# scaleoutsystems/multimodal-MoE

Hardware: AMD Instinct MI355X
Metric: images/sec (fwd+bwd) RT-DETR-MoE 1280×720 bs=8/GPU at 1/2/4/8 MI355X (higher is better)
Workload: dtype bf16; 1 GPU; C2: RT-DETR-R50 + 8-expert top-2 MoE, bs=8/GPU, bf16; arch=rtdetr-r50-moe8-top2, global_batch=8, execution=hipGraph: forward + criterion (GPU matcher) + backward, precision=bf16 weights + fp32 master, img=1280x720 (padded to 1280x736), parallelism=dp1, batch=8

## Files before the change

### include/moe_hip.h

```cpp
#ifndef MOE_HIP_H_
#define MOE_HIP_H_

#include <stdint.h>
#include <hip/hip_runtime_api.h>

#ifdef __cplusplus
extern "C" {
#endif

int moe_router_num_blocks(int T);

int moe_router_topk_fwd(const void* x, const float* wg, const float* ctx_bias,
                        const int32_t* ctx_img, int n_ctx, int tokens_per_image,
                        int T, int d, int E, int k, int normalize,
                        int32_t* topk_idx, float* topk_w, float* probs, float* lse,
                        int32_t* local_rank, int32_t* block_counts,
                        float* aux_partials, hipStream_t stream);

int moe_route_scan(const int32_t* block_counts, int nblk, int k, int E, int cap,
                   int32_t* rank_base, int32_t* hist, int32_t* offsets,
                   hipStream_t stream);

int moe_permute_fwd(const void* x, const int32_t* topk_idx, const int32_t* local_rank,
                    const int32_t* rank_base, const int32_t* offsets,
// ... 298 lines not shown
int rtdetr_conv_fwd_act(const void* x, const void* w, void* y, const void* zero, int B, int H, int W, int C, int N,
                        int KS, int stride, const float* bias, const void* resid, int act, int resid_post,
                        long long y_img_rows, long long y_row_off, hipStream_t stream);
int rtdetr_conv_fwd_stats_rows(int B, int H, int W, int C, int N, int KS, int stride);
int rtdetr_conv_fwd_stats(const void* x, const void* w, void* y, const void* zero, int B, int H, int W, int C,
                          int N, int KS, int stride, float* part, hipStream_t stream);
long long rtdetr_conv_dgrad_workspace(int B, int H, int W, int C, int N, int KS);
int rtdetr_conv_dgrad(const void* dy, const void* w, void* work, void* dx, const void* zero, int B, int H, int W,
                      int C, int N, int KS, int stride, const void* add, const void* relu_mask, hipStream_t stream);
int rtdetr_conv_weight_flip_multi(const void* table, int n, int total_blocks, hipStream_t stream);
int rtdetr_conv_dgrad_preflipped(const void* dy, const void* w, const void* wflip, void* dx, const void* zero, int B,
                                 int H, int W, int C, int N, int KS, int stride, const void* add, const void* relu_mask,
                                 hipStream_t stream);
int rtdetr_conv_wgrad_splits(int B, int H, int W, int C, int N, int KS);
int rtdetr_conv_wgrad(const void* dy, const void* x, float* part, int nsplit, void* dw, int out_bf16,
                      const void* zero, int B, int H, int W, int C, int N, int KS, int stride, hipStream_t stream);
int rtdetr_conv_wgrad_part(const void* dy, const void* x, float* part, int nsplit, const void* zero, int B, int H,
                           int W, int C, int N, int KS, int stride, hipStream_t stream);
int rtdetr_conv_wgrad_reduce_batch(int n, const float* const* parts, const int* nsplits, const long long* nws,
                                   void* const* dws, int out_bf16, hipStream_t stream);
int rtdetr_conv1x1_bwd(const void* dy, const void* x, const void* w, void* dx, float* part, int nsplit,
                       const void* zero, int B, int H, int W, int C, int N, const void* add, int mask_input,
                       hipStream_t stream);
int rtdetr_conv_set_tuning(const char* key, int value);

int train_grad_pack(const void* tensors, const int32_t* chunks, int n_chunks, float* flat, hipStream_t stream);
int train_grad_sqnorm(const void* tensors, const int32_t* chunks, int n_chunks, float* partials,
                      hipStream_t stream);
int train_grad_norm_finalize(const float* partials, int n, float max_norm, float inv_world, float* coef,
                             const void* tensors, int n_tensors, int32_t* tensor_steps, hipStream_t stream);
int train_adamw_step(const void* tensors, const int32_t* chunks, int n_chunks, const float* coef,
                     float* master, float* exp_avg, float* exp_avg_sq, const int32_t* tensor_steps,
                     const float* lrs, int n_groups, float weight_decay, float beta1, float beta2, float eps,
                     hipStream_t stream);

int train_adamw_ema_step(const void* tensors, const int32_t* chunks, int n_chunks, const float* coef,
                         float* master, float* exp_avg, float* exp_avg_sq, const int32_t* tensor_steps,
                         const float* lrs, int n_groups, float weight_decay, float beta1, float beta2, float eps,
                         float* ema, float ema_decay, hipStream_t stream);
int train_ema_update(const void* tensors, const int32_t* chunks, int n_chunks, float* ema, float ema_decay,
                     hipStream_t stream);

int train_grad_accum(const void* tensors, const int32_t* chunks, int n_chunks, float* acc, int first,
                     hipStream_t stream);

int train_augment_images(const void* src, int src_dtype, long long sn, long long sc, long long sh, long long sw,
// ... 53 lines not shown
```

### multimodal-moe_amd/csrc/conv.hip

```cpp
#include <algorithm>

#include "mfma_lds.h"
#include "moe_common.h"
#include "prof.h"

namespace moe {

static int wg_bm(int N) { return N % 128 == 0 ? 128 : 64; }
static int wg_bn(int C) { return C % 128 == 0 ? 128 : 64; }
static int g_conv_bm = 0;
static int g_conv_big = 0;
static int g_conv_wg_stages = 0;
static int g_conv_wg_splits = 0;
static int g_conv_dgrad_flip = -1;
static int g_conv_dgrad_phase = 1;
static int g_conv_areg = 0;
static int g_conv_halo = -1;
static int g_conv_8ph = -1;
static int g_conv_k32 = -1;

struct ConvArgs {
  const uint16_t* x;
  const uint16_t* w;
  uint16_t* y;
// ... 1242 lines not shown
          const uint32_t lo = mw[q] & 0xffffu, hi = mw[q] >> 16;
          const uint32_t keep_lo = ((lo & 0x8000u) || lo == 0) ? 0u : 0xffffu;
          const uint32_t keep_hi = ((hi & 0x8000u) || hi == 0) ? 0u : 0xffff0000u;
          vw[q] &= keep_lo | keep_hi;
        }
        v = make_uint4(vw[0], vw[1], vw[2], vw[3]);
      }
      const long long p = p0 + r;
      if (p < a.P) *reinterpret_cast<uint4*>(a.dx + (size_t)p * C + xs * 64 + (lane & 7) * 8) = v;
    }
    rslot = rslot + 1 == S ? 0 : rslot + 1;
    islot = islot + 1 == S ? 0 : islot + 1;
  }
#pragma unroll
  for (int i = 0; i < 4; ++i) {
    float* row = out + (size_t)(64 * nb + 16 * i + (lane & 15)) * C + 64 * cb + 4 * (lane >> 4);
#pragma unroll
    for (int j = 0; j < 4; ++j)
      *reinterpret_cast<float4*>(row + 16 * j) =
          make_float4(accw[i][j][0], accw[i][j][1], accw[i][j][2], accw[i][j][3]);
  }
}

template <auto FN>
static void allow_lds_once(size_t bytes) {
  static unsigned long long done = 0;
  (void)allow_dyn_lds(reinterpret_cast<const void*>(FN), (int)bytes, &done, "conv: dynamic LDS");
}

static int conv_out(int n, int KS, int stride) { return (n + 2 * ((KS - 1) / 2) - KS) / stride + 1; }

static int conv_check(const void* const* ptrs, int np, int B, int H, int W, int C, int N, int KS, int stride,
                      const char* what, int cmul = 64) {
  if (KS != 1 && KS != 3) return fail(std::string(what) + ": kernel size must be 1 or 3");
  if (stride != 1 && !(stride == 2 && KS == 3)) return fail(std::string(what) + ": stride must be 1 (or 2 with KS 3)");
  if (B < 0 || H <= 0 || W <= 0) return fail(std::string(what) + ": bad B / H / W");
  if (C % cmul || N % cmul || C <= 0 || N <= 0)
    return fail(std::string(what) + ": channels must be positive multiples of " + std::to_string(cmul));
  if ((long long)B * H * W * (C > N ? C : N) >= (1ll << 31)) return fail(std::string(what) + ": tensor too large");
  for (int i = 0; i < np; ++i)
    if (ptrs[i] == nullptr || reinterpret_cast<uintptr_t>(ptrs[i]) % 16)
      return fail(std::string(what) + ": operands must be non-NULL and 16-B aligned");
  return 0;
}

constexpr int CV_STAGES = 2;
// ... 448 lines not shown
  if (int rc = conv_check(ptrs, 6, B, H, W, C, N, 1, 1, "rtdetr_conv1x1_bwd")) return rc;
  if (!((C == 64 && N == 256) || (C == 256 && N == 64)))
    return fail("rtdetr_conv1x1_bwd: takes {C, N} = {64, 256} (the ResNet stage-1 1x1 layers)");
  if (!aligned16(add)) return fail("rtdetr_conv1x1_bwd: add must be 16-B aligned");
  if (nsplit < 1 || nsplit > 256) return fail("rtdetr_conv1x1_bwd: nsplit must be 1..256");
  Conv1x1BwdArgs a{static_cast<const uint16_t*>(dy), static_cast<const uint16_t*>(x), static_cast<const uint16_t*>(w),
                   static_cast<uint16_t*>(dx), part, static_cast<const uint16_t*>(add),
                   static_cast<const uint16_t*>(zero), B * H * W, 0, mask_input ? 1 : 0};
  const int ktot = (a.P + 63) / 64;
  a.kt_per = (ktot + nsplit - 1) / nsplit;
  const double P = a.P, nw = (double)N * C;
  ProfScope prof(stream, PROF_CONV, 2.0 * P * (N + 2 * C + (add ? C : 0)) + 2.0 * nw + 4.0 * nsplit * nw, false, 0.0,
                 4.0 * P * nw);
  if (C == 64) {
    if (add) launch_conv1x1_bwd<64, 256, true>(a, nsplit, stream, prof);
    else launch_conv1x1_bwd<64, 256, false>(a, nsplit, stream, prof);
  } else {
    if (add) launch_conv1x1_bwd<256, 64, true>(a, nsplit, stream, prof);
    else launch_conv1x1_bwd<256, 64, false>(a, nsplit, stream, prof);
  }
  return check_launch("rtdetr_conv1x1_bwd");
}

extern "C" int rtdetr_conv3x3_direct_fwd(const void* x, const float* wf, const float* bias, void* y, int B, int H,
                                         int W, int C, int N, int stride, int relu, hipStream_t stream) {
  if (C != 3 || N != 32) return fail("rtdetr_conv3x3_direct_fwd: takes C = 3 -> N = 32 (the ResNet-D stem)");
  if (stride != 1 && stride != 2) return fail("rtdetr_conv3x3_direct_fwd: stride 1 or 2");
  if (B < 0 || H <= 0 || W <= 0) return fail("rtdetr_conv3x3_direct_fwd: bad B / H / W");
  if (B == 0) return 0;
  if (x == nullptr || wf == nullptr || y == nullptr || reinterpret_cast<uintptr_t>(y) % 16)
    return fail("rtdetr_conv3x3_direct_fwd: x, wf non-NULL, y 16-B aligned");
  const int Ho = conv_out(H, 3, stride), Wo = conv_out(W, 3, stride);
  const long long P = (long long)B * Ho * Wo;
  const long long blocks = (P + 255) / 256;
  if (blocks > 0x7fffffffLL) return fail("rtdetr_conv3x3_direct_fwd: too many pixels");
  ProfScope prof(stream, PROF_CONV, 2.0 * ((double)B * H * W * C + P * N), false, 0.0, 2.0 * P * N * 9 * C);
  MOE_LAUNCH(prof, (conv_direct_kernel<32, 3>), dim3((unsigned)blocks), dim3(256), 0, stream,
             static_cast<const uint16_t*>(x), wf, bias, static_cast<uint16_t*>(y), B, H, W, Ho, Wo, stride, relu);
  return check_launch("rtdetr_conv3x3_direct_fwd");
}

extern "C" int rtdetr_conv_set_tuning(const char* key, int value) {
  if (key == nullptr) return fail("rtdetr_conv_set_tuning: key is NULL");
  if (std::string(key) == "conv_bm") {
    g_conv_bm = value;
    return 0;
// ... 41 lines not shown
```

### multimodal-moe_amd/src/moe/_lib.py

```python
from __future__ import annotations

import ctypes
import os
from pathlib import Path

import torch

_PKG = Path(__file__).resolve().parents[2]
LIB_PATH = Path(os.environ.get("MOE_HIP_LIB", _PKG / "lib" / "libmoe_hip.so"))

MOE_BF16 = 0
MOE_FP8_E4M3 = 1
MOE_BIAS_BF16 = 0x100
MOE_DENSE_LAYER = 0x200
EPI_NONE, EPI_BIAS, EPI_BIAS_RELU, EPI_RELU_MASK, EPI_RELU_MASK_MX = 0, 1, 2, 3, 4
MX_BLOCK = 32

_P = ctypes.c_void_p
_I = ctypes.c_int
_F = ctypes.c_float
_LL = ctypes.c_longlong
SIGNATURES = {
    "moe_router_num_blocks": (_I, [_I]),
    "moe_router_topk_fwd": (_I, [_P, _P, _P, _P, _I, _I, _I, _I, _I, _I, _I, _P, _P, _P, _P, _P, _P, _P, _P]),
# ... 93 lines not shown
                             _I, _I, _I, _I, _F, _P]),
    "rtdetr_attn_fwd_seg": (_I, [_P, _LL, _P, _LL, _P, _LL, _P, _LL, _P, _I, _I, _I, _I, _F, _P, _P]),
    "rtdetr_attn_bwd_seg": (_I, [_P, _LL, _P, _LL, _P, _LL, _P, _LL, _P, _LL, _P, _P, _P, _LL, _P, _LL, _P, _LL,
                                 _I, _I, _I, _I, _F, _P, _P]),
    "rtdetr_conv_fwd": (_I, [_P, _P, _P, _P, _I, _I, _I, _I, _I, _I, _I, _P, _P, _I, _P]),
    "rtdetr_conv_fwd_act": (_I, [_P, _P, _P, _P, _I, _I, _I, _I, _I, _I, _I, _P, _P, _I, _I, _LL, _LL, _P]),
    "rtdetr_conv_fwd_stats_rows": (_I, [_I, _I, _I, _I, _I, _I, _I]),
    "rtdetr_conv_fwd_stats": (_I, [_P, _P, _P, _P, _I, _I, _I, _I, _I, _I, _I, _P, _P]),
    "rtdetr_bn_act_fwd_part": (_I, [_P, _P, _P, _P, _P, _I, ctypes.c_longlong, _I, _I, _F, _F, _P, _I, _P, _P, _P]),
    "rtdetr_bn_act_fwd_rows": (_I, [_P, _P, _P, _P, _P, _I, ctypes.c_longlong, _I, _I, _F, _F, _P, _I, _P, _P, _P,
                                    _P, ctypes.c_longlong, ctypes.c_longlong, _P]),
    "rtdetr_bn_act_bwd_rows": (_I, [_P, ctypes.c_longlong, ctypes.c_longlong, _P, _P, _I, ctypes.c_longlong, _I, _I,
                                    _P, _P, _P, _P, _P, _P]),
    "rtdetr_conv_dgrad_workspace": (_LL, [_I, _I, _I, _I, _I, _I]),
    "rtdetr_conv_dgrad": (_I, [_P, _P, _P, _P, _P, _I, _I, _I, _I, _I, _I, _I, _P, _P, _P]),
    "rtdetr_conv_dgrad_preflipped": (_I, [_P, _P, _P, _P, _P, _I, _I, _I, _I, _I, _I, _I, _P, _P, _P]),
    "rtdetr_conv_weight_flip_multi": (_I, [_P, _I, _I, _P]),
    "rtdetr_conv_wgrad_splits": (_I, [_I, _I, _I, _I, _I, _I]),
    "rtdetr_conv_set_tuning": (_I, [ctypes.c_char_p, _I]),
    "rtdetr_conv_wgrad": (_I, [_P, _P, _P, _I, _P, _I, _P, _I, _I, _I, _I, _I, _I, _I, _P]),
    "rtdetr_conv_wgrad_part": (_I, [_P, _P, _P, _I, _P, _I, _I, _I, _I, _I, _I, _I, _P]),
    "rtdetr_conv_wgrad_reduce_batch": (_I, [_I, _P, _P, _P, _P, _I, _P]),
    "rtdetr_conv1x1_bwd": (_I, [_P, _P, _P, _P, _P, _I, _P, _I, _I, _I, _I, _I, _P, _I, _P]),
    "train_grad_pack": (_I, [_P, _P, _I, _P, _P]),
    "train_grad_accum": (_I, [_P, _P, _I, _P, _I, _P]),
    "train_grad_sqnorm": (_I, [_P, _P, _I, _P, _P]),
    "train_grad_norm_finalize": (_I, [_P, _I, _F, _F, _P, _P, _I, _P, _P]),
    "train_adamw_step": (_I, [_P, _P, _I, _P, _P, _P, _P, _P, _P, _I, _F, _F, _F, _F, _P]),
    "train_adamw_ema_step": (_I, [_P, _P, _I, _P, _P, _P, _P, _P, _P, _I, _F, _F, _F, _F, _P, _F, _P]),
    "train_ema_update": (_I, [_P, _P, _I, _P, _F, _P]),
    "train_augment_images": (_I, [_P, _I, _LL, _LL, _LL, _LL, _P, _I, _P, _I, _I, _I, _I, _I, _F, _P]),
    "train_augment_boxes": (_I, [_P, _P, _P, _P, _I, _I, _I, _I, _I, _I, _P, _P, _P, _P, _P]),
    "train_mosaic_images": (_I, [_P, _I, _LL, _LL, _LL, _LL, _I, _P, _I, _P, _I, _I, _I, _I, _I, _F, _P]),
    "train_mosaic_boxes": (_I, [_P, _P, _P, _P, _I, _I, _I, _I, _I, _I, _I, _P, _P, _P, _P, _P]),
    "moe_profile_enable": (_I, [_I]),
    "moe_profile_count": (_I, []),
    "moe_profile_get": (_I, [_I, _P, _P, _P, _P]),
    "moe_profile_clear": (_I, []),
    "moe_expert_ffn_bwd": (_I, [_P, _P, _P, _P, _P, _P, _P, _P, _I, _I, _I, _I, _P, _P, _P, _P, _P, _P, _I, _P]),
    "moe_launch_counts": (_I, [_P, _I]),
    "moe_launch_counts_reset": (_I, []),
    "moe_last_error": (ctypes.c_char_p, []),
    "moe_version": (ctypes.c_char_p, []),
}


# ... 1343 lines not shown
```

### multimodal-moe_amd/src/rtdetr_moe/backbone.py

```python
from __future__ import annotations

import ctypes
import os

import torch
from torch import nn
import torch.nn.functional as F

from .conv import conv2d, conv2d_add_bias_relu_fork, conv2d_bias_relu, conv_module, conv_module_stats, hip_conv_ok_for
from .fused import AddBiasReLU, AddBiasReLUFork, BiasReLU, bn_act, bn_act_eval, bn_act_ok, bn_eval_ok

_FUSED_BN = os.environ.get("MOE_FUSED_BN", "1") != "0"
_FUSED_EPI = os.environ.get("MOE_CONV_EPI", "1") != "0"

_DEPTHS = {18: [2, 2, 2, 2], 34: [3, 4, 6, 3], 50: [3, 4, 6, 3], 101: [3, 4, 23, 3]}


class FrozenBatchNorm2d(nn.Module):

    def __init__(self, n, eps=1e-5):
        super().__init__()
        self.register_buffer("weight", torch.ones(n))
        self.register_buffer("bias", torch.zeros(n))
        self.register_buffer("running_mean", torch.zeros(n))
        self.register_buffer("running_var", torch.ones(n))
        self.eps = eps

    def scale_shift(self):
        key = (self.weight.device, self.weight._version, self.bias._version, self.running_mean._version,
               self.running_var._version)
        cache = getattr(self, "_ss_cache", None)
        if cache is None or cache[0] != key:
# ... 136 lines not shown
        L = self.lib
        L._check(L.lib().rtdetr_fold_scale_multi(self.table.data_ptr(), self.chunks.data_ptr(), self.n_chunks,
                                                 L._stream()), "rtdetr_fold_scale_multi")


class ConvNormLayer(nn.Module):

    def __init__(self, cin, cout, k, s, act=None, frozen=False):
        super().__init__()
        self.conv = nn.Conv2d(cin, cout, k, s, (k - 1) // 2, bias=False)
        self.norm = _norm(cout, frozen)
        self.act_name = act
        self.act = nn.ReLU(inplace=True) if act == "relu" else (nn.SiLU(inplace=True) if act == "silu" else nn.Identity())
        self.fold = frozen and act in (None, "relu")

    def folded(self):
        scale, shift = self.norm.scale_shift()
        w = getattr(self, "_w_folded", None)
        self._w_folded = None
        if w is None:
            w = _FoldScale.apply(self.conv.weight, scale)
        return w, shift

    def conv_shift(self, x, folded=None):
        w, shift = folded if folded is not None else self.folded()
        return conv2d(x, w, self.conv.stride, self.conv.padding), shift

    def hip_ok(self, x_like, cin, w):
        return (_FUSED_EPI and self.fold and x_like.shape[0] > 0
                and hip_conv_ok_for(x_like.is_cuda, x_like.dtype, cin, w, self.conv.stride, self.conv.padding))

    def bias_relu(self, x, folded, mask_input=False, grad_premasked=False, link=None):
        w, shift = folded
        if mask_input or grad_premasked or self.hip_ok(x, x.shape[1], w):
            return conv2d_bias_relu(x, w, shift, mask_input, grad_premasked, link, self.conv.stride)
        y, _ = self.conv_shift(x, folded)
        return BiasReLU.apply(y, shift)

    def forward(self, x):
        if self.fold:
            y, shift = self.conv_shift(x)
            if self.act_name == "relu":
                return BiasReLU.apply(y, shift)
            return y + shift.view(1, -1, 1, 1).to(y.dtype)
        if self.act_name in (None, "silu") and _FUSED_BN:
            if not self.norm.training and not torch.is_grad_enabled():
                from . import evalfold

                y = evalfold.conv_folded(self, x)
                if y is not None:
                    return y
                y = conv_module(self.conv, x)
                if bn_eval_ok([y], [self.norm]):
                    return bn_act_eval([y], [self.norm], self.act_name)
                return self.act(self.norm(y))
            y, part = conv_module_stats(self.conv, x)
            if bn_act_ok([y], [self.norm]):
                return bn_act([y], [self.norm], self.act_name, part)
# ... 108 lines not shown

class _Shortcut(nn.Module):

    def __init__(self, cin, cout, stride, frozen):
        super().__init__()
        self.down = stride == 2
        self.conv = ConvNormLayer(cin, cout, 1, 1, frozen=frozen)

    def forward(self, x):
        return self.conv(avg_pool_2x2(x) if self.down else x)

    def conv_shift(self, x, link=None):
        return self.conv.conv_shift(avg_pool_2x2(x, link) if self.down else x)


_NO_FORK = os.environ.get("MOE_BACKBONE_FORK", "1") == "0"
_NO_FOLD_ALL = os.environ.get("MOE_FOLD_ALL", "1") == "0"


def _fork_ok(short):
    return not _NO_FORK and (short is None or short.conv.fold)


def _block_out(last, short, h, x, folded_last=None, mask_input=False, link_in=None, short_link=None):
    if last.fold and _fork_ok(short) and folded_last is not None:
        wl, sl = folded_last
        if mask_input or last.hip_ok(h, h.shape[1], wl):
            b, bias = (x, sl) if short is None else short.conv_shift(x, short_link)
            if short is not None:
                bias = sl + bias
            return conv2d_add_bias_relu_fork(h, wl, b, bias, mask_input, link_in if short is None else None)
    if mask_input:
        raise RuntimeError("_block_out: mask_input set but the fused fork path does not run")
    if last.fold and (short is None or short.conv.fold):
        a, sa = last.conv_shift(h, folded_last)
        b, bias = (x, sa) if short is None else short.conv_shift(x)
        if short is not None:
            bias = sa + bias
        if _NO_FORK:
            y = AddBiasReLU.apply(a, b, bias)
            return y, y
        return AddBiasReLUFork.apply(a, b, bias)
    y = F.relu(last(h) + (x if short is None else short(x)))
    return y, y


_GRAD_LINK = os.environ.get("MOE_GRAD_LINK", "1") != "0"


_DOWN_LINK = os.environ.get("MOE_DOWN_LINK", "1") != "0"


def _link_for(short, x, fused):
    if not fused or not _GRAD_LINK:
        return None
    if short is not None and not (_DOWN_LINK and short.down and short.conv.fold):
        return None
    return getattr(x, "grad_link", None)


class BasicBlock(nn.Module):
    expansion = 1

    def __init__(self, cin, cout, stride, shortcut, frozen):
        super().__init__()
        self.short = None if shortcut else _Shortcut(cin, cout, stride, frozen)
        self.branch2a = ConvNormLayer(cin, cout, 3, stride, "relu", frozen)
        self.branch2b = ConvNormLayer(cout, cout, 3, 1, None, frozen)

    def forward(self, x, x_short=None):
        xs = x if x_short is None else x_short
        a, b = self.branch2a, self.branch2b
        if _FUSED_EPI and a.fold and b.fold and a.act_name == "relu" and x.is_cuda:
            fa, fb = a.folded(), b.folded()
            ok_a = a.hip_ok(x, x.shape[1], fa[0])
            ok_b = b.hip_ok(x, fa[0].shape[0], fb[0]) and _fork_ok(self.short)
            pre_ab = ok_a and ok_b
            link = _link_for(self.short, x, ok_a and ok_b)
            h = a.bias_relu(x, fa, grad_premasked=pre_ab, link=link) if ok_a else a.bias_relu(x, fa)
            return _block_out(b, self.short, h, xs, fb, mask_input=pre_ab, link_in=link)
        return _block_out(self.branch2b, self.short, self.branch2a(x), xs)


class BottleNeck(nn.Module):
    expansion = 4

    def __init__(self, cin, cout, stride, shortcut, frozen):
        super().__init__()
        width = cout
        self.branch2a = ConvNormLayer(cin, width, 1, 1, "relu", frozen)
        self.branch2b = ConvNormLayer(width, width, 3, stride, "relu", frozen)
        self.branch2c = ConvNormLayer(width, cout * 4, 1, 1, None, frozen)
        self.short = None if shortcut else _Shortcut(cin, cout * 4, stride, frozen)

    def forward(self, x, x_short=None):
        xs = x if x_short is None else x_short
        a, b, c = self.branch2a, self.branch2b, self.branch2c
        if _FUSED_EPI and a.fold and b.fold and c.fold and x.is_cuda:
            fa, fb, fc = a.folded(), b.folded(), c.folded()
            ok_a = a.hip_ok(x, x.shape[1], fa[0])
            ok_b = b.hip_ok(x, fa[0].shape[0], fb[0])
            ok_c = c.hip_ok(x, fb[0].shape[0], fc[0]) and _fork_ok(self.short)
            pre_ab, pre_bc = ok_a and ok_b, ok_b and ok_c
            link = _link_for(self.short, x, ok_a and ok_c)
            h1 = a.bias_relu(x, fa, grad_premasked=pre_ab, link=link)
            h2 = b.bias_relu(h1, fb, mask_input=pre_ab, grad_premasked=pre_bc)
            return _block_out(c, self.short, h2, xs, fc, mask_input=pre_bc, link_in=link,
                              short_link=link if self.short is not None else None)
        return _block_out(self.branch2c, self.short, self.branch2b(self.branch2a(x)), xs)


class PResNet(nn.Module):
    def __init__(self, depth=50, return_idx=(1, 2, 3), freeze_norm=True, freeze_at=0):
        super().__init__()
        block = BottleNeck if depth >= 50 else BasicBlock
        c = 64
        self.stem = nn.Sequential(
            ConvNormLayer(3, c // 2, 3, 2, "relu", freeze_norm),
            ConvNormLayer(c // 2, c // 2, 3, 1, "relu", freeze_norm),
            ConvNormLayer(c // 2, c, 3, 1, "relu", freeze_norm),
        )
        self.pool = nn.MaxPool2d(3, 2, 1)
        ch_in = c
        self.stages = nn.ModuleList()
        self.out_channels = []
        for i, (n, cout) in enumerate(zip(_DEPTHS[depth], [64, 128, 256, 512])):
            stride = 1 if i == 0 else 2
            blocks = []
            for b in range(n):
                shortcut = b > 0 or (i == 0 and block is BasicBlock)
                blocks.append(block(ch_in, cout, stride if b == 0 else 1, shortcut, freeze_norm))
# ... 43 lines not shown
        if not self._stem_hip_ok(x):
            return self.stem(x)
        from ..moe import _lib as L
        from .conv import _fwd, _nhwc

        l1, l2, l3 = self.stem
        if x.dtype != torch.bfloat16:
            x = x.to(torch.bfloat16).contiguous(memory_format=torch.channels_last)
        w, shift = l1.folded()
        y = L.conv3x3_direct_fwd(x, w.to(torch.bfloat16), shift.float().contiguous(), l1.conv.stride[0], True)
        for l in (l2, l3):
            if _STEM_HIP >= 2:
                w, shift = l.folded()
                y = _fwd(y, _nhwc(w.to(torch.bfloat16)), shift.float().contiguous(), None, True, l.conv.stride[0])
            else:
                y = l(y)
        return y

    def forward(self, x):
        self._fold_all()
        x = stem_max_pool(self._stem(x), self.pool)
        xs = None
        outs = []
        for i, stage in enumerate(self.stages):
            for blk in stage:
                x, xs = blk(x, xs)
            if i in self.return_idx:
                outs.append(x)
        return stage_taps(outs)


@torch.no_grad()
def calibrate_frozen_bn(model: nn.Module, images: torch.Tensor, residual_gain: float | None = 0.1) -> int:
    layers = [m for m in model.modules() if isinstance(m, ConvNormLayer) and isinstance(m.norm, FrozenBatchNorm2d)]
    if residual_gain is not None:
        for blk in model.modules():
            last = getattr(blk, "branch2c", None) if isinstance(blk, BottleNeck) else \
                (getattr(blk, "branch2b", None) if isinstance(blk, BasicBlock) else None)
            if last is not None and isinstance(last.norm, FrozenBatchNorm2d):
                last.norm.weight.fill_(residual_gain)

    def pre(mod, args):
        x = args[0]
        y = F.conv2d(x, mod.conv.weight.to(x.dtype), None, mod.conv.stride, mod.conv.padding).float()
        mod.norm.running_mean.copy_(y.mean((0, 2, 3)))
        mod.norm.running_var.copy_(y.var((0, 2, 3), unbiased=False))
        mod._w_folded = None

    global _FUSED_EPI
# ... 21 lines not shown
```

### multimodal-moe_amd/src/rtdetr_moe/conv.py

```python
from __future__ import annotations

import os

import torch
import torch.nn.functional as F

_ENABLED = [os.environ.get("MOE_HIP_CONV", "1") != "0"]
_ZERO = {}


def _zero(dev):
    z = _ZERO.get(dev)
    if z is None:
        z = _ZERO[dev] = torch.zeros(256, dtype=torch.bfloat16, device=dev)
    return z


def _nhwc(t):
    return t if t.is_contiguous(memory_format=torch.channels_last) else t.contiguous(memory_format=torch.channels_last)


def hip_conv_ok(x, w, stride=1, padding=None, dilation=1, groups=1) -> bool:
    if not (x.dim() == 4 and x.shape[0] > 0):
        return False
# ... 13 lines not shown
            and cin == C and C % 64 == 0 and N % 64 == 0)


def _stride(stride) -> int:
    return stride if isinstance(stride, int) else stride[0]


def _out(n, ks, st):
    return (n + 2 * ((ks - 1) // 2) - ks) // st + 1


def _fwd(x, w, bias=None, resid=None, relu=False, st=1):
    from ..moe import _lib as L

    B, C, H, W = x.shape
    N, _, ks, _ = w.shape
    y = torch.empty((B, N, _out(H, ks, st), _out(W, ks, st)), dtype=torch.bfloat16, device=x.device,
                    memory_format=torch.channels_last)
    L._check(L.lib().rtdetr_conv_fwd(x.data_ptr(), w.data_ptr(), y.data_ptr(), _zero(x.device).data_ptr(),
                                     B, H, W, C, N, ks, st, None if bias is None else bias.data_ptr(),
                                     None if resid is None else resid.data_ptr(), int(relu), L._stream()),
             "rtdetr_conv_fwd")
    return y


def conv_act_eval(x, w, bias, act, resid=None, st=1, out=None, out_row=0):
    from ..moe import _lib as L

    x = _nhwc(x)
    if x.data_ptr() % 16:
        x = x.clone(memory_format=torch.channels_last)
    if resid is not None:
        resid = _nhwc(resid)
        if resid.data_ptr() % 16:
            resid = resid.clone(memory_format=torch.channels_last)
    B, C, H, W = x.shape
    N, _, ks, _ = w.shape
    Ho, Wo = _out(H, ks, st), _out(W, ks, st)
    if out is not None:
        if resid is not None or not (out.dim() == 3 and out.shape[0] == B and out.shape[2] == N
                                     and out.dtype == torch.bfloat16 and out.is_contiguous()
                                     and 0 <= out_row and out_row + Ho * Wo <= out.shape[1]):
            raise ValueError("conv_act_eval: out must be a contiguous bf16 [B, S, N] holding the rows")
        y, rows = out, out.shape[1]
    else:
        y = torch.empty((B, N, Ho, Wo), dtype=torch.bfloat16, device=x.device, memory_format=torch.channels_last)
# ... 190 lines not shown
    _reduce_wgrads(pend, L._stream())
    pend.clear()


def _reduce_wgrads(pend, s):
    import ctypes

    from ..moe import _lib as L

    for i in range(0, len(pend), _WG_BATCH):
        chunk = pend[i:i + _WG_BATCH]
        n = len(chunk)
        parts = (ctypes.c_void_p * n)(*[c[0].data_ptr() for c in chunk])
        nsplit = (ctypes.c_int * n)(*[c[1] for c in chunk])
        numel = (ctypes.c_longlong * n)(*[c[2] for c in chunk])
        dws = (ctypes.c_void_p * n)(*[c[3].data_ptr() for c in chunk])
        cv = lambda a: ctypes.cast(a, ctypes.c_void_p)
        L._check(L.lib().rtdetr_conv_wgrad_reduce_batch(n, cv(parts), cv(nsplit), cv(numel), cv(dws), 1, s),
                 "rtdetr_conv_wgrad_reduce_batch")


class GradLink:

    __slots__ = ("g_short", "final", "g_ext", "ext_used")

    def __init__(self):
        self.g_short = None
        self.final = False
        self.g_ext = None
        self.ext_used = False


class _ConvHIP(torch.autograd.Function):

    @staticmethod
    def forward(ctx, x, w, bias=None, relu=False, mask_input=False, grad_premasked=False, link=None, st=1):
        x = _nhwc(x)
        w = _nhwc(w)
        y = _fwd(x, w, bias, None, relu, st)
        ctx.st = st
        ctx.flags = (bool(relu) and not grad_premasked, bool(mask_input))
        ctx.link = link
        ctx.save_for_backward(x, w, y if ctx.flags[0] else None)
        return y

    @staticmethod
    def backward(ctx, gy):
        x, w, y = ctx.saved_tensors
        relu_here, mask_input = ctx.flags
        g = torch.ops.aten.threshold_backward(gy, y, 0) if relu_here else gy
        link, add = ctx.link, None
        if link is not None and link.g_short is not None and ctx.needs_input_grad[0]:
            add, mask_input = link.g_short, True
            link.g_short, link.final = None, True
        gx, gw = _bwd(x, w, g, ctx.needs_input_grad[0], ctx.needs_input_grad[1], mask_input, add, ctx.st)
        return gx, gw, None, None, None, None, None, None


class _ConvHIPFork(torch.autograd.Function):

    @staticmethod
    def forward(ctx, x, w, resid, bias, mask_input=False, link_in=None, link_out=None):
        x = _nhwc(x)
        w = _nhwc(w)
        y = _fwd(x, w, bias, _nhwc(resid), True)
        ctx.set_materialize_grads(False)
        ctx.mask_input = bool(mask_input)
        ctx.links = (link_in, link_out)
        ctx.save_for_backward(x, w, y)
        return y, y.view_as(y)

    @staticmethod
    def backward(ctx, dy1, dy2):
        from ..moe import _lib as L

        x, w, y = ctx.saved_tensors
        link_in, link_out = ctx.links
        ext = None
        if link_out is not None:
            if link_out.g_ext is not None and not link_out.ext_used:
                ext = link_out.g_ext
            link_out.g_ext, link_out.ext_used = None, False
        if link_out is not None and link_out.final:
            g = dy1
            link_out.final = False
            if ext is not None:
                g = g + torch.where(y > 0, ext, torch.zeros_like(ext))
        else:
            if link_out is not None:
                link_out.g_short = None
            if ext is not None:
                dy1 = ext if dy1 is None else dy1 + ext
            if dy1 is None and dy2 is None:
                return None, None, None, None, None, None, None
            if dy1 is None:
                dy1, dy2 = dy2, None
            g = L.relu_grad2_nhwc(_nhwc(dy1), None if dy2 is None else _nhwc(dy2), y)
        if link_in is not None:
            link_in.g_short = g
        gx, gw = _bwd(x, w, g, ctx.needs_input_grad[0], ctx.needs_input_grad[1], ctx.mask_input)
        return gx, gw, g if ctx.needs_input_grad[2] else None, None, None, None, None


class GradSlot:

    __slots__ = ("g", "closed", "has_collector", "__weakref__")

    def __init__(self):
        self.g = None
        self.closed = False
        self.has_collector = False
        _OPEN_SLOTS.append(self)
        if len(_OPEN_SLOTS) > 256:
            del _OPEN_SLOTS[:128]


_OPEN_SLOTS: list = []


def check_grad_slots():
    pending = [s for s in _OPEN_SLOTS if s.g is not None]
    _OPEN_SLOTS.clear()
    if pending:
        for s in pending:
# ... 95 lines not shown


_PAIR_ON = os.environ.get("MOE_CONV_PAIR", "1") != "0"
_STATS_ON = os.environ.get("MOE_CONV_BN_STATS", "1") != "0"


def _autocast_operands(x, w, stride, padding, dilation=1, groups=1):
    if (x.is_cuda and x.dim() == 4 and x.shape[0] > 0 and torch.is_autocast_enabled("cuda")
            and torch.get_autocast_dtype("cuda") == torch.bfloat16
            and x.dtype in (torch.float32, torch.bfloat16) and w.dtype in (torch.float32, torch.bfloat16)
            and hip_conv_ok_for(True, torch.bfloat16, x.shape[1], w, stride, padding, dilation, groups,
                                w_dtype=torch.bfloat16)):
        return x.to(torch.bfloat16), w.to(torch.bfloat16)
    return x, w


def conv2d(x, weight, stride=1, padding=0):
    xc, wc = _autocast_operands(x, weight, stride, padding)
    if hip_conv_ok(xc, wc, stride, padding):
        return _ConvHIP.apply(xc, wc, None, False, False, False, None, _stride(stride))
    return F.conv2d(x, weight, None, stride, padding)


def conv2d_bias_relu(x, weight, bias, mask_input=False, grad_premasked=False, link=None, stride=1):
    return _ConvHIP.apply(x, weight, bias.float().contiguous(), True, mask_input, grad_premasked, link,
                          _stride(stride))


def conv2d_add_bias_relu_fork(x, weight, resid, bias, mask_input=False, link_in=None):
    link_out = GradLink()
    y, y2 = _ConvHIPFork.apply(x, weight, resid, None if bias is None else bias.float().contiguous(), mask_input,
                               link_in, link_out)
    y.grad_link = link_out
    return y, y2


def conv_module(conv: torch.nn.Conv2d, x):
    if conv.bias is None:
        xc, wc = _autocast_operands(x, conv.weight, conv.stride, conv.padding, conv.dilation, conv.groups)
        if hip_conv_ok(xc, wc, conv.stride, conv.padding, conv.dilation, conv.groups):
            return _ConvHIP.apply(xc, wc, None, False, False, False, None, _stride(conv.stride))
    return conv(x)
```

Before: 355.6 images/sec.

## Fuse bottleneck output conv with shortcut conv and next block's branch2a

Adds a HIP kernel that computes the bottleneck's final 1x1 conv (64->256), adds either the residual tensor or a fused 1x1 shortcut conv, applies bias and ReLU, and optionally runs the next block's 1x1 branch2a conv (256->64/128) on the output tile while it is still in LDS. The next block then picks up the parked result instead of launching its own conv. The aim is to cut kernel launches and the HBM round trips for the residual, the shortcut output and the re-read of the block output in the ResNet-50 stage-1 forward. In exchange it adds version-checked parking logic in Python and a new backward path for the fused shortcut, and it only applies to stage-1 shapes.

```diff
diff --git a/include/moe_hip.h b/include/moe_hip.h
--- a/include/moe_hip.h
+++ b/include/moe_hip.h
@@ -344,6 +344,9 @@
 int rtdetr_conv1x1_bwd(const void* dy, const void* x, const void* w, void* dx, float* part, int nsplit,
                        const void* zero, int B, int H, int W, int C, int N, const void* add, int mask_input,
                        hipStream_t stream);
+int rtdetr_conv1x1_block_out(const void* h2, const void* w2c, const void* resid, const void* xs, const void* ws,
+                             const float* bias, void* y, const void* wn, const float* bias_n, void* h, int next,
+                             const void* zero, int B, int H, int W, int nwg, hipStream_t stream);
 int rtdetr_conv_set_tuning(const char* key, int value);
 
 int train_grad_pack(const void* tensors, const int32_t* chunks, int n_chunks, float* flat, hipStream_t stream);
diff --git a/multimodal-moe_amd/csrc/conv.hip b/multimodal-moe_amd/csrc/conv.hip
--- a/multimodal-moe_amd/csrc/conv.hip
+++ b/multimodal-moe_amd/csrc/conv.hip
@@ -1288,6 +1288,248 @@
   }
 }
 
+struct BlockOutArgs {
+  const uint16_t* h2;
+  const uint16_t* w2c;
+  const uint16_t* res;
+  const uint16_t* ws;
+  const float* bias;
+  uint16_t* y;
+  const uint16_t* wn;
+  const float* bias_n;
+  uint16_t* h;
+  const uint16_t* zero;
+  int P, kt_per;
+};
+
+template <bool RC>
+struct BlockOutCfg {
+  static constexpr int RS = RC ? 1 : 4;
+  static constexpr int S = RC ? 6 : 3;
+  static constexpr int SUB = 64 * 128;
+  static constexpr int STAGE = (1 + RS) * SUB;
+  static constexpr int GW = 2 * (1 + RS);
+  static constexpr int YOFF = S * STAGE;
+  static constexpr int HOFF = YOFF + (RC ? 4 * SUB : 0);
+  static constexpr size_t lds(int next) { return HOFF + (size_t)(next / 64) * SUB; }
+};
+
+__device__ __forceinline__ void unpack2(uint32_t w, float& lo, float& hi) {
+  lo = __uint_as_float(w << 16);
+  hi = __uint_as_float(w & 0xffff0000u);
+}
+
+template <bool RC, int NEXT>
+__global__ __launch_bounds__(256) void stage1_out_kernel(BlockOutArgs a) {
+  extern __shared__ __attribute__((aligned(16))) char smem[];
+  static_assert(NEXT == 0 || NEXT == 64 || NEXT == 128, "next branch2a: none, 64 or 128 channels");
+  using Cfg = BlockOutCfg<RC>;
+  constexpr int RS = Cfg::RS, S = Cfg::S, SUB = Cfg::SUB, STAGE = Cfg::STAGE, GW = Cfg::GW;
+  static_assert((S - 2) * GW <= 63, "vmcnt range");
+  constexpr int TN2 = NEXT / 64;
+  constexpr int T2 = TN2 > 0 ? TN2 : 1;
+  const int tid = threadIdx.x, lane = tid & 63;
+  const int wave = __builtin_amdgcn_readfirstlane(tid >> 6);
+  const int ktot = (a.P + 63) / 64;
+  const int kt0 = blockIdx.x * a.kt_per;
+  const int nk = max(0, min(a.kt_per, ktot - kt0));
+  if (nk == 0) return;
+  const int frow = lane & 15, fk = 8 * (lane >> 4);
+  bf16x8 wc[4][2], wsf[RC ? 4 : 1][2], wnf[T2][8];
+  float bi[4][4], bn[T2][4];
+#pragma unroll
+  for (int j = 0; j < 4; ++j) {
+    const int n = 64 * wave + 16 * j;
+#pragma unroll
+    for (int ks = 0; ks < 2; ++ks) {
+      wc[j][ks] = *reinterpret_cast<const bf16x8*>(a.w2c + (size_t)(n + frow) * 64 + 32 * ks + fk);
+      if constexpr (RC) wsf[j][ks] = *reinterpret_cast<const bf16x8*>(a.ws + (size_t)(n + frow) * 64 + 32 * ks + fk);
+    }
+    const float4 b = *reinterpret_cast<const float4*>(a.bias + n + 4 * (lane >> 4));
+    bi[j][0] = b.x; bi[j][1] = b.y; bi[j][2] = b.z; bi[j][3] = b.w;
+  }
+  if constexpr (NEXT > 0) {
+#pragma unroll
+    for (int j = 0; j < TN2; ++j) {
+      const int n = (NEXT / 4) * wave + 16 * j;
+#pragma unroll
+      for (int k8 = 0; k8 < 8; ++k8)
+        wnf[j][k8] = *reinterpret_cast<const bf16x8*>(a.wn + (size_t)(n + frow) * 256 + 32 * k8 + fk);
+      const float4 b = *reinterpret_cast<const float4*>(a.bias_n + n + 4 * (lane >> 4));
+      bn[j][0] = b.x; bn[j][1] = b.y; bn[j][2] = b.z; bn[j][3] = b.w;
+    }
+  }
+#pragma unroll
+  for (int j = 0; j < 4; ++j)
+#pragma unroll
+    for (int ks = 0; ks < 2; ++ks) {
+      asm volatile("" : "+v"(wc[j][ks]));
+      if constexpr (RC) asm volatile("" : "+v"(wsf[j][ks]));
+    }
+  if constexpr (NEXT > 0) {
+#pragma unroll
+    for (int j = 0; j < TN2; ++j)
+#pragma unroll
+      for (int k8 = 0; k8 < 8; ++k8) asm volatile("" : "+v"(wnf[j][k8]));
+  }
+  wait_vm<0>();
+  const int rowA = 8 * wave + (lane >> 3);
+  const int c8 = ((lane & 7) ^ sub_swz(rowA)) * 8;
+  auto issue = [&](int kt, int slot) {
+    char* buf = smem + slot * STAGE;
+    const long long p0 = (long long)(kt0 + kt) * 64 + rowA;
+#pragma unroll
+    for (int j = 0; j < GW; ++j) {
+      const int sub = j >> 1;
+      const long long p = p0 + 32 * (j & 1);
+      const uint16_t* src = sub == 0 ? a.h2 + (size_t)p * 64 + c8
+                                     : a.res + (size_t)p * (64 * RS) + (sub - 1) * 64 + c8;
+      dma16_uncounted(p < a.P ? src : a.zero + c8, buf + sub * SUB + (wave + 4 * (j & 1)) * 1024);
+    }
+  };
+#pragma unroll
+  for (int s = 0; s < S - 1; ++s)
+    if (s < nk) issue(s, s);
+  char* const hst = smem + Cfg::HOFF;
+  int rslot = 0, islot = S - 1;
+  for (int kt = 0; kt < nk; ++kt) {
+    {
+      const int newer = min(S - 2, nk - 1 - kt);
+      if (newer >= 4) wait_vm<(S >= 6 ? 4 : 0) * GW>();
+      else if (newer == 3) wait_vm<(S >= 5 ? 3 : 0) * GW>();
+      else if (newer == 2) wait_vm<(S >= 4 ? 2 : 0) * GW>();
+      else if (newer == 1) wait_vm<(S >= 3 ? 1 : 0) * GW>();
+      else wait_vm<0>();
+    }
+    asm volatile("s_waitcnt lgkmcnt(0)" ::: "memory");
+    __builtin_amdgcn_s_barrier();
+    char* cur = smem + rslot * STAGE;
+    char* yimg = RC ? smem + Cfg::YOFF : cur + SUB;
+    const long long p0 = (long long)(kt0 + kt) * 64;
+    if (kt + S - 1 < nk) issue(kt + S - 1, islot);
+    f32x4 acc[4][4], accs[RC ? 4 : 1][RC ? 4 : 1];
+#pragma unroll
+    for (int i = 0; i < 4; ++i)
+#pragma unroll
+      for (int j = 0; j < 4; ++j) {
+        acc[i][j] = f32x4{0.f, 0.f, 0.f, 0.f};
+        if constexpr (RC) accs[i][j] = f32x4{0.f, 0.f, 0.f, 0.f};
+      }
+#pragma unroll
+    for (int ks = 0; ks < 2; ++ks) {
+      bf16x8 af[4];
+#pragma unroll
+      for (int i = 0; i < 4; ++i) af[i] = sub_frag_k(cur, 16 * i, ks, lane);
+#pragma unroll
+      for (int i = 0; i < 4; ++i)
+#pragma unroll
+        for (int j = 0; j < 4; ++j)
+          acc[i][j] = __builtin_amdgcn_mfma_f32_16x16x32_bf16(wc[j][ks], af[i], acc[i][j], 0, 0, 0);
+      if constexpr (RC) {
+#pragma unroll
+        for (int i = 0; i < 4; ++i) af[i] = sub_frag_k(cur + SUB, 16 * i, ks, lane);
+#pragma unroll
+        for (int i = 0; i < 4; ++i)
+#pragma unroll
+          for (int j = 0; j < 4; ++j)
+            accs[i][j] = __builtin_amdgcn_mfma_f32_16x16x32_bf16(wsf[j][ks], af[i], accs[i][j], 0, 0, 0);
+      }
+    }
+    char* ysub = yimg + wave * SUB;
+#pragma unroll
+    for (int i = 0; i < 4; ++i) {
+      const int r = 16 * i + (lane & 15);
+#pragma unroll
+      for (int j = 0; j < 4; ++j) {
+        const int col = 16 * j + 4 * (lane >> 4);
+        uint2* at = reinterpret_cast<uint2*>(ysub + sub_off(r, col >> 3) + (col & 7) * 2);
+        uint2 q;
+        if constexpr (RC) {
+          q.x = pack2bf(accs[i][j][0], accs[i][j][1]);
+          q.y = pack2bf(accs[i][j][2], accs[i][j][3]);
+        } else {
+          q = *at;
+        }
+        float f[4], g[4];
+        unpack2(pack2bf(acc[i][j][0], acc[i][j][1]), f[0], f[1]);
+        unpack2(pack2bf(acc[i][j][2], acc[i][j][3]), f[2], f[3]);
+        unpack2(q.x, g[0], g[1]);
+        unpack2(q.y, g[2], g[3]);
+#pragma unroll
+        for (int e = 0; e < 4; ++e) {
+          f[e] += g[e];
+          f[e] += bi[j][e];
+          f[e] = fmaxf(f[e], 0.f);
+        }
+        uint2 v;
+        v.x = pack2bf(f[0], f[1]);
+        v.y = pack2bf(f[2], f[3]);
+        *at = v;
+      }
+    }
+#pragma unroll
+    for (int e = 0; e < 8; ++e) {
+      const int r = (lane >> 3) + 8 * e;
+      const uint4 v = *reinterpret_cast<const uint4*>(ysub + sub_off(r, lane & 7));
+      const long long p = p0 + r;
+      if (p < a.P) *reinterpret_cast<uint4*>(a.y + (size_t)p * 256 + 64 * wave + (lane & 7) * 8) = v;
+    }
+    if constexpr (NEXT > 0) {
+      asm volatile("s_waitcnt lgkmcnt(0)" ::: "memory");
+      __builtin_amdgcn_s_barrier();
+      f32x4 acc2[4][T2];
+#pragma unroll
+      for (int i = 0; i < 4; ++i)
+#pragma unroll
+        for (int j = 0; j < TN2; ++j) acc2[i][j] = f32x4{0.f, 0.f, 0.f, 0.f};
+#pragma unroll
+      for (int k8 = 0; k8 < 8; ++k8) {
+        bf16x8 af[4];
+#pragma unroll
+        for (int i = 0; i < 4; ++i) af[i] = sub_frag_k(yimg + (k8 >> 1) * SUB, 16 * i, k8 & 1, lane);
+#pragma unroll
+        for (int i = 0; i < 4; ++i)
+#pragma unroll
+          for (int j = 0; j < TN2; ++j)
+            acc2[i][j] = __builtin_amdgcn_mfma_f32_16x16x32_bf16(wnf[j][k8], af[i], acc2[i][j], 0, 0, 0);
+      }
+#pragma unroll
+      for (int i = 0; i < 4; ++i) {
+        const int r = 16 * i + (lane & 15);
+#pragma unroll
+        for (int j = 0; j < TN2; ++j) {
+          const int col = (NEXT / 4) * wave + 16 * j + 4 * (lane >> 4);
+          float f[4];
+          unpack2(pack2bf(acc2[i][j][0], acc2[i][j][1]), f[0], f[1]);
+          unpack2(pack2bf(acc2[i][j][2], acc2[i][j][3]), f[2], f[3]);
+#pragma unroll
+          for (int e = 0; e < 4; ++e) {
+            f[e] += bn[j][e];
+            f[e] = fmaxf(f[e], 0.f);
+          }
+          uint2 v;
+          v.x = pack2bf(f[0], f[1]);
+          v.y = pack2bf(f[2], f[3]);
+          *reinterpret_cast<uint2*>(hst + (col >> 6) * SUB + sub_off(r, (col & 63) >> 3) + (col & 7) * 2) = v;
+        }
+      }
+      asm volatile("s_waitcnt lgkmcnt(0)" ::: "memory");
+      __builtin_amdgcn_s_barrier();
+      constexpr int CPRN = NEXT / 8;
+#pragma unroll
+      for (int e = 0; e < NEXT / 32; ++e) {
+        const int idx = tid + 256 * e;
+        const int r = idx / CPRN, c = idx % CPRN;
+        const uint4 v = *reinterpret_cast<const uint4*>(hst + (c >> 3) * SUB + sub_off(r, c & 7));
+        const long long p = p0 + r;
+        if (p < a.P) *reinterpret_cast<uint4*>(a.h + (size_t)p * NEXT + c * 8) = v;
+      }
+    }
+    rslot = rslot + 1 == S ? 0 : rslot + 1;
+    islot = islot + 1 == S ? 0 : islot + 1;
+  }
+}
+
 template <auto FN>
 static void allow_lds_once(size_t bytes) {
   static unsigned long long done = 0;
@@ -1782,6 +2024,55 @@
   return check_launch("rtdetr_conv1x1_bwd");
 }
 
+template <bool RC, int NEXT>
+static void launch_block_out(const BlockOutArgs& a, int grid, hipStream_t stream, ProfScope& prof) {
+  constexpr size_t lds = BlockOutCfg<RC>::lds(NEXT);
+  static_assert(lds <= 160 * 1024, "ring + tiles exceed the CU's LDS");
+  allow_lds_once<stage1_out_kernel<RC, NEXT>>(lds);
+  MOE_LAUNCH(prof, (stage1_out_kernel<RC, NEXT>), dim3(grid), dim3(256), lds, stream, a);
+}
+
+extern "C" int rtdetr_conv1x1_block_out(const void* h2, const void* w2c, const void* resid, const void* xs,
+                                        const void* ws, const float* bias, void* y, const void* wn,
+                                        const float* bias_n, void* h, int next, const void* zero, int B, int H, int W,
+                                        int nwg, hipStream_t stream) {
+  const char* what = "rtdetr_conv1x1_block_out";
+  const void* ptrs[5] = {h2, w2c, bias, y, zero};
+  if (int rc = conv_check(ptrs, 5, B, H, W, 64, 256, 1, 1, what)) return rc;
+  if ((resid != nullptr) == (xs != nullptr)) return fail(std::string(what) + ": give resid or (xs, ws), not both");
+  if (xs != nullptr && ws == nullptr) return fail(std::string(what) + ": xs without ws");
+  if (next != 0 && next != 64 && next != 128) return fail(std::string(what) + ": next must be 0, 64 or 128");
+  if (next != 0 && (wn == nullptr || bias_n == nullptr || h == nullptr))
+    return fail(std::string(what) + ": next without wn / bias_n / h");
+  if (!aligned16(resid) || !aligned16(xs) || !aligned16(ws) || !aligned16(wn) || !aligned16(bias_n) || !aligned16(h))
+    return fail(std::string(what) + ": operands must be 16-B aligned");
+  if (nwg < 0) return fail(std::string(what) + ": nwg must be >= 0 (0 = automatic)");
+  if (B == 0) return 0;
+  const bool rc_ = xs != nullptr;
+  BlockOutArgs a{static_cast<const uint16_t*>(h2), static_cast<const uint16_t*>(w2c),
+                 static_cast<const uint16_t*>(rc_ ? xs : resid), static_cast<const uint16_t*>(ws), bias,
+                 static_cast<uint16_t*>(y), static_cast<const uint16_t*>(wn), bias_n, static_cast<uint16_t*>(h),
+                 static_cast<const uint16_t*>(zero), B * H * W, 0};
+  const int ktot = (a.P + 63) / 64;
+  const int want = std::min(ktot, nwg > 0 ? nwg : 256);
+  a.kt_per = (ktot + want - 1) / want;
+  const int grid = (ktot + a.kt_per - 1) / a.kt_per;
+  const double P = a.P;
+  ProfScope prof(stream, PROF_CONV,
+                 2.0 * P * (64 + (rc_ ? 64 : 256) + 256 + next) + 2.0 * 64 * 256 * (rc_ ? 2 : 1) + 2.0 * next * 256,
+                 false, 0.0, 2.0 * P * 256 * (64.0 * (rc_ ? 2 : 1) + next));
+  if (rc_) {
+    if (next == 0) launch_block_out<true, 0>(a, grid, stream, prof);
+    else if (next == 64) launch_block_out<true, 64>(a, grid, stream, prof);
+    else launch_block_out<true, 128>(a, grid, stream, prof);
+  } else {
+    if (next == 0) launch_block_out<false, 0>(a, grid, stream, prof);
+    else if (next == 64) launch_block_out<false, 64>(a, grid, stream, prof);
+    else launch_block_out<false, 128>(a, grid, stream, prof);
+  }
+  return check_launch(what);
+}
+
 extern "C" int rtdetr_conv3x3_direct_fwd(const void* x, const float* wf, const float* bias, void* y, int B, int H,
                                          int W, int C, int N, int stride, int relu, hipStream_t stream) {
   if (C != 3 || N != 32) return fail("rtdetr_conv3x3_direct_fwd: takes C = 3 -> N = 32 (the ResNet-D stem)");
diff --git a/multimodal-moe_amd/src/moe/_lib.py b/multimodal-moe_amd/src/moe/_lib.py
--- a/multimodal-moe_amd/src/moe/_lib.py
+++ b/multimodal-moe_amd/src/moe/_lib.py
@@ -139,6 +139,7 @@
     "rtdetr_conv_wgrad_part": (_I, [_P, _P, _P, _I, _P, _I, _I, _I, _I, _I, _I, _I, _P]),
     "rtdetr_conv_wgrad_reduce_batch": (_I, [_I, _P, _P, _P, _P, _I, _P]),
     "rtdetr_conv1x1_bwd": (_I, [_P, _P, _P, _P, _P, _I, _P, _I, _I, _I, _I, _I, _P, _I, _P]),
+    "rtdetr_conv1x1_block_out": (_I, [_P, _P, _P, _P, _P, _P, _P, _P, _P, _P, _I, _P, _I, _I, _I, _I, _P]),
     "train_grad_pack": (_I, [_P, _P, _I, _P, _P]),
     "train_grad_accum": (_I, [_P, _P, _I, _P, _I, _P]),
     "train_grad_sqnorm": (_I, [_P, _P, _I, _P, _P]),
diff --git a/multimodal-moe_amd/src/rtdetr_moe/backbone.py b/multimodal-moe_amd/src/rtdetr_moe/backbone.py
--- a/multimodal-moe_amd/src/rtdetr_moe/backbone.py
+++ b/multimodal-moe_amd/src/rtdetr_moe/backbone.py
@@ -7,7 +7,8 @@
 from torch import nn
 import torch.nn.functional as F
 
-from .conv import conv2d, conv2d_add_bias_relu_fork, conv2d_bias_relu, conv_module, conv_module_stats, hip_conv_ok_for
+from .conv import (chain_short_ok, conv2d, conv2d_add_bias_relu_fork, conv2d_bias_relu,
+                   conv2d_short_add_bias_relu_fork, conv_module, conv_module_stats, hip_conv_ok_for, take_parked)
 from .fused import AddBiasReLU, AddBiasReLUFork, BiasReLU, bn_act, bn_act_eval, bn_act_ok, bn_eval_ok
 
 _FUSED_BN = os.environ.get("MOE_FUSED_BN", "1") != "0"
@@ -190,6 +191,12 @@
             w = _FoldScale.apply(self.conv.weight, scale)
         return w, shift
 
+    def peek_folded(self):
+        w = getattr(self, "_w_folded", None)
+        if w is None or not self.fold:
+            return None
+        return w, self.norm.scale_shift()[1]
+
     def conv_shift(self, x, folded=None):
         w, shift = folded if folded is not None else self.folded()
         return conv2d(x, w, self.conv.stride, self.conv.padding), shift
@@ -201,7 +208,8 @@
     def bias_relu(self, x, folded, mask_input=False, grad_premasked=False, link=None):
         w, shift = folded
         if mask_input or grad_premasked or self.hip_ok(x, x.shape[1], w):
-            return conv2d_bias_relu(x, w, shift, mask_input, grad_premasked, link, self.conv.stride)
+            out = take_parked(x, folded) if self.conv.kernel_size == (1, 1) else None
+            return conv2d_bias_relu(x, w, shift, mask_input, grad_premasked, link, self.conv.stride, out)
         y, _ = self.conv_shift(x, folded)
         return BiasReLU.apply(y, shift)
 
@@ -356,14 +364,19 @@
     return not _NO_FORK and (short is None or short.conv.fold)
 
 
-def _block_out(last, short, h, x, folded_last=None, mask_input=False, link_in=None, short_link=None):
+def _block_out(last, short, h, x, folded_last=None, mask_input=False, link_in=None, short_link=None, next_a=None):
     if last.fold and _fork_ok(short) and folded_last is not None:
         wl, sl = folded_last
         if mask_input or last.hip_ok(h, h.shape[1], wl):
+            nxt = next_a.peek_folded() if next_a is not None and next_a.act_name == "relu" else None
+            if short is not None and not short.down and short.conv.fold and short.conv.conv.stride == (1, 1):
+                if chain_short_ok(h, wl, x, short.conv.conv.weight):
+                    ws, ss = short.conv.folded()
+                    return conv2d_short_add_bias_relu_fork(h, wl, x, ws, sl + ss, mask_input, nxt)
             b, bias = (x, sl) if short is None else short.conv_shift(x, short_link)
             if short is not None:
                 bias = sl + bias
-            return conv2d_add_bias_relu_fork(h, wl, b, bias, mask_input, link_in if short is None else None)
+            return conv2d_add_bias_relu_fork(h, wl, b, bias, mask_input, link_in if short is None else None, nxt)
     if mask_input:
         raise RuntimeError("_block_out: mask_input set but the fused fork path does not run")
     if last.fold and (short is None or short.conv.fold):
@@ -402,7 +415,7 @@
         self.branch2a = ConvNormLayer(cin, cout, 3, stride, "relu", frozen)
         self.branch2b = ConvNormLayer(cout, cout, 3, 1, None, frozen)
 
-    def forward(self, x, x_short=None):
+    def forward(self, x, x_short=None, next_a=None):
         xs = x if x_short is None else x_short
         a, b = self.branch2a, self.branch2b
         if _FUSED_EPI and a.fold and b.fold and a.act_name == "relu" and x.is_cuda:
@@ -427,7 +440,7 @@
         self.branch2c = ConvNormLayer(width, cout * 4, 1, 1, None, frozen)
         self.short = None if shortcut else _Shortcut(cin, cout * 4, stride, frozen)
 
-    def forward(self, x, x_short=None):
+    def forward(self, x, x_short=None, next_a=None):
         xs = x if x_short is None else x_short
         a, b, c = self.branch2a, self.branch2b, self.branch2c
         if _FUSED_EPI and a.fold and b.fold and c.fold and x.is_cuda:
@@ -440,7 +453,7 @@
             h1 = a.bias_relu(x, fa, grad_premasked=pre_ab, link=link)
             h2 = b.bias_relu(h1, fb, mask_input=pre_ab, grad_premasked=pre_bc)
             return _block_out(c, self.short, h2, xs, fc, mask_input=pre_bc, link_in=link,
-                              short_link=link if self.short is not None else None)
+                              short_link=link if self.short is not None else None, next_a=next_a)
         return _block_out(self.branch2c, self.short, self.branch2b(self.branch2a(x)), xs)
 
 
@@ -530,9 +543,11 @@
         x = stem_max_pool(self._stem(x), self.pool)
         xs = None
         outs = []
+        blocks = [blk for stage in self.stages for blk in stage]
+        nexts = iter([getattr(b, "branch2a", None) for b in blocks[1:]] + [None])
         for i, stage in enumerate(self.stages):
             for blk in stage:
-                x, xs = blk(x, xs)
+                x, xs = blk(x, xs, next(nexts))
             if i in self.return_idx:
                 outs.append(x)
         return stage_taps(outs)
diff --git a/multimodal-moe_amd/src/rtdetr_moe/conv.py b/multimodal-moe_amd/src/rtdetr_moe/conv.py
--- a/multimodal-moe_amd/src/rtdetr_moe/conv.py
+++ b/multimodal-moe_amd/src/rtdetr_moe/conv.py
@@ -59,6 +59,62 @@
                                      None if resid is None else resid.data_ptr(), int(relu), L._stream()),
              "rtdetr_conv_fwd")
     return y
+
+
+_CHAIN_ON = os.environ.get("MOE_CONV_CHAIN", "1") != "0"
+
+
+def _chain_ok(x, w, bias) -> bool:
+    return (_CHAIN_ON and bias is not None and x.is_cuda and x.dim() == 4 and x.shape[0] > 0 and x.shape[1] == 64
+            and x.dtype == torch.bfloat16 and w.dtype == torch.bfloat16 and tuple(w.shape) == (256, 64, 1, 1))
+
+
+def _chain_next_ok(nxt) -> bool:
+    if nxt is None:
+        return False
+    wn = nxt[0]
+    return (wn.is_cuda and wn.dtype == torch.bfloat16 and wn.dim() == 4 and tuple(wn.shape[1:]) == (256, 1, 1)
+            and wn.shape[0] in (64, 128) and wn.data_ptr() % 16 == 0)
+
+
+def _fwd_block_out(x, w, bias, resid=None, xs=None, ws=None, nxt=None):
+    from ..moe import _lib as L
+
+    B, _, H, W = x.shape
+    y = torch.empty((B, 256, H, W), dtype=torch.bfloat16, device=x.device, memory_format=torch.channels_last)
+    h = wn = bn = None
+    if nxt is not None:
+        wn, bn = nxt
+        h = torch.empty((B, wn.shape[0], H, W), dtype=torch.bfloat16, device=x.device,
+                        memory_format=torch.channels_last)
+    p = lambda t: None if t is None else t.data_ptr()
+    L._check(L.lib().rtdetr_conv1x1_block_out(x.data_ptr(), w.data_ptr(), p(resid), p(xs), p(ws), bias.data_ptr(),
+                                              y.data_ptr(), p(wn), p(bn), p(h), 0 if wn is None else wn.shape[0],
+                                              _zero(x.device).data_ptr(), B, H, W, 0, L._stream()),
+             "rtdetr_conv1x1_block_out")
+    return y, h
+
+
+def _park_next(link, h, nxt):
+    if h is not None:
+        wn, shift = nxt
+        link.h_next = (h, wn, wn._version, shift, shift._version)
+
+
+def take_parked(x, folded):
+    link = getattr(x, "grad_link", None)
+    p = getattr(link, "h_next", None) if link is not None else None
+    if p is None:
+        return None
+    link.h_next = None
+    h, wn, vw, sn, vs = p
+    w, shift = folded
+    same_w = w is wn or (w.data_ptr() == wn.data_ptr() and w.shape == wn.shape and w.dtype == wn.dtype
+                         and w.stride() == wn.stride())
+    if same_w and w._version == vw and shift is sn and shift._version == vs and h.shape[0] == x.shape[0] \
+            and h.shape[2:] == x.shape[2:]:
+        return h
+    return None
 
 
 def conv_act_eval(x, w, bias, act, resid=None, st=1, out=None, out_row=0):
@@ -295,9 +351,10 @@
 
 class GradLink:
 
-    __slots__ = ("g_short", "final", "g_ext", "ext_used")
+    __slots__ = ("g_short", "final", "g_ext", "ext_used", "h_next")
 
     def __init__(self):
+        self.h_next = None
         self.g_short = None
         self.final = False
         self.g_ext = None
@@ -307,10 +364,10 @@
 class _ConvHIP(torch.autograd.Function):
 
     @staticmethod
-    def forward(ctx, x, w, bias=None, relu=False, mask_input=False, grad_premasked=False, link=None, st=1):
+    def forward(ctx, x, w, bias=None, relu=False, mask_input=False, grad_premasked=False, link=None, st=1, out=None):
         x = _nhwc(x)
         w = _nhwc(w)
-        y = _fwd(x, w, bias, None, relu, st)
+        y = out if out is not None else _fwd(x, w, bias, None, relu, st)
         ctx.st = st
         ctx.flags = (bool(relu) and not grad_premasked, bool(mask_input))
         ctx.link = link
@@ -327,16 +384,20 @@
             add, mask_input = link.g_short, True
             link.g_short, link.final = None, True
         gx, gw = _bwd(x, w, g, ctx.needs_input_grad[0], ctx.needs_input_grad[1], mask_input, add, ctx.st)
-        return gx, gw, None, None, None, None, None, None
+        return gx, gw, None, None, None, None, None, None, None
 
 
 class _ConvHIPFork(torch.autograd.Function):
 
     @staticmethod
-    def forward(ctx, x, w, resid, bias, mask_input=False, link_in=None, link_out=None):
+    def forward(ctx, x, w, resid, bias, mask_input=False, link_in=None, link_out=None, nxt=None):
         x = _nhwc(x)
         w = _nhwc(w)
-        y = _fwd(x, w, bias, _nhwc(resid), True)
+        if nxt is not None:
+            y, h = _fwd_block_out(x, w, bias, resid=_nhwc(resid), nxt=(nxt[0], nxt[1].float().contiguous()))
+            _park_next(link_out, h, nxt)
+        else:
+            y = _fwd(x, w, bias, _nhwc(resid), True)
         ctx.set_materialize_grads(False)
         ctx.mask_input = bool(mask_input)
         ctx.links = (link_in, link_out)
@@ -365,14 +426,59 @@
             if ext is not None:
                 dy1 = ext if dy1 is None else dy1 + ext
             if dy1 is None and dy2 is None:
-                return None, None, None, None, None, None, None
+                return None, None, None, None, None, None, None, None
             if dy1 is None:
                 dy1, dy2 = dy2, None
             g = L.relu_grad2_nhwc(_nhwc(dy1), None if dy2 is None else _nhwc(dy2), y)
         if link_in is not None:
             link_in.g_short = g
         gx, gw = _bwd(x, w, g, ctx.needs_input_grad[0], ctx.needs_input_grad[1], ctx.mask_input)
-        return gx, gw, g if ctx.needs_input_grad[2] else None, None, None, None, None
+        return gx, gw, g if ctx.needs_input_grad[2] else None, None, None, None, None, None
+
+
+class _ConvHIPForkShort(torch.autograd.Function):
+
+    @staticmethod
+    def forward(ctx, x, w, xs, ws, bias, mask_input=False, link_out=None, nxt=None):
+        x, xs = _nhwc(x), _nhwc(xs)
+        w, ws = _nhwc(w), _nhwc(ws)
+        y, h = _fwd_block_out(x, w, bias, xs=xs, ws=ws,
+                              nxt=None if nxt is None else (nxt[0], nxt[1].float().contiguous()))
+        _park_next(link_out, h, nxt)
+        ctx.set_materialize_grads(False)
+        ctx.mask_input = bool(mask_input)
+        ctx.link_out = link_out
+        ctx.save_for_backward(x, w, xs, ws, y)
+        return y, y.view_as(y)
+
+    @staticmethod
+    def backward(ctx, dy1, dy2):
+        from ..moe import _lib as L
+
+        x, w, xs, ws, y = ctx.saved_tensors
+        link_out = ctx.link_out
+        ext = None
+        if link_out.g_ext is not None and not link_out.ext_used:
+            ext = link_out.g_ext
+        link_out.g_ext, link_out.ext_used = None, False
+        if link_out.final:
+            g = dy1
+            link_out.final = False
+            if ext is not None:
+                g = g + torch.where(y > 0, ext, torch.zeros_like(ext))
+        else:
+            link_out.g_short = None
+            if ext is not None:
+                dy1 = ext if dy1 is None else dy1 + ext
+            if dy1 is None and dy2 is None:
+                return None, None, None, None, None, None, None, None
+            if dy1 is None:
+                dy1, dy2 = dy2, None
+            g = L.relu_grad2_nhwc(_nhwc(dy1), None if dy2 is None else _nhwc(dy2), y)
+        need = ctx.needs_input_grad
+        gx, gw = _bwd(x, w, g, need[0], need[1], ctx.mask_input)
+        gxs, gws = _bwd(xs, ws, g, need[2], need[3], False)
+        return gx, gw, gxs, gws, None, None, None, None
 
 
 class GradSlot:
@@ -514,15 +620,32 @@
     return F.conv2d(x, weight, None, stride, padding)
 
 
-def conv2d_bias_relu(x, weight, bias, mask_input=False, grad_premasked=False, link=None, stride=1):
+def conv2d_bias_relu(x, weight, bias, mask_input=False, grad_premasked=False, link=None, stride=1, out=None):
     return _ConvHIP.apply(x, weight, bias.float().contiguous(), True, mask_input, grad_premasked, link,
-                          _stride(stride))
-
-
-def conv2d_add_bias_relu_fork(x, weight, resid, bias, mask_input=False, link_in=None):
+                          _stride(stride), out)
+
+
+def conv2d_add_bias_relu_fork(x, weight, resid, bias, mask_input=False, link_in=None, nxt=None):
     link_out = GradLink()
-    y, y2 = _ConvHIPFork.apply(x, weight, resid, None if bias is None else bias.float().contiguous(), mask_input,
-                               link_in, link_out)
+    bias = None if bias is None else bias.float().contiguous()
+    if not (_chain_ok(x, weight, bias) and _chain_next_ok(nxt) and resid.dtype == torch.bfloat16
+            and tuple(resid.shape) == (x.shape[0], 256) + tuple(x.shape[2:])):
+        nxt = None
+    y, y2 = _ConvHIPFork.apply(x, weight, resid, bias, mask_input, link_in, link_out, nxt)
+    y.grad_link = link_out
+    return y, y2
+
+
+def chain_short_ok(x, weight, xs, ws) -> bool:
+    return (_chain_ok(x, weight, True) and xs.is_cuda and xs.dtype == torch.bfloat16 and ws.dtype == torch.bfloat16
+            and tuple(ws.shape) == (256, 64, 1, 1) and tuple(xs.shape) == tuple(x.shape)
+            and not (torch.is_autocast_enabled("cuda") and xs.dtype != torch.get_autocast_dtype("cuda")))
+
+
+def conv2d_short_add_bias_relu_fork(x, weight, xs, ws, bias, mask_input=False, nxt=None):
+    link_out = GradLink()
+    y, y2 = _ConvHIPForkShort.apply(x, weight, xs, ws, bias.float().contiguous(), mask_input, link_out,
+                                    nxt if _chain_next_ok(nxt) else None)
     y.grad_link = link_out
     return y, y2
 
```

Result: faster. 359.4 images/sec (median of 6 runs) (+1.1%).
